# mees/hulc2

Measured on AMD Instinct MI355X. Metric: play-sequences/sec/node (seq_len=32, 200x200 RGB), higher is better.
Workload: dtype bf16; 1 GPU; BASELINE configs[1]: synthetic CALVIN-shaped batch, Hulc2.training_step fwd+bwd+allreduce+Adam, static CNN 200x200 + gripper CNN 84x84, lang = random (B,384) embeddings, dropout 0.1, gripper_control on; sequences_per_gpu_step=64, seq_len=32, parallelism=dp1, launch=hipGraph replay (fwd+bwd graph, all-reduce, optimizer graph), frames=fp32 NCHW, already transformed (the reference's dataloader output), gradient_allreduce=none (one rank, no process group), exact_forward_sites=encfc,goal,head,txl

## Files before the change

### hulc2_amd/csrc/conv_band.h

```cpp
#pragma once
#include "hulc_common.h"

namespace hulc_band {

#define BAND_MAXCLS 4
struct BandCls {
    int OH, OW;
    long y_off;
    int co_base;
    long w_row0;
    long w_tap_off[16];
};
struct BandP {
    const void* X; void* Y; const void* Wt; const float* bias; const void* mask;
    const void* add;
    void* Y16;
    int x_dtype, y_dtype, w_dtype, mask_dtype;
    int Nimg, H, W;
    int OHmax, OWmax;
    int pad_y, pad_x;
    int R;
    int F;
    long x_sn, x_sy, x_sx;
    long y_sn, y_sy, y_sx;
    long ldw;
    int relu;
    unsigned* bits_out;
    const unsigned* bits_in;
    int bshift; long bplane;
    BandCls cls[BAND_MAXCLS];
};

HULC_DEVICE uint4 band_load_bits(const void* X, long off) { return *(const uint4*)((const uint16_t*)X + off); }
template <bool XF32>
HULC_DEVICE uint4 band_load_x(const void* X, long off) {
    if (!XF32) return band_load_bits(X, off);
    const float4* q = (const float4*)((const float*)X + off);
    const float4 a = q[0], c = q[1];
    return make_uint4(pack_bf16x2(a.x, a.y), pack_bf16x2(a.z, a.w), pack_bf16x2(c.x, c.y), pack_bf16x2(c.z, c.w));
}

int launch_band_planes(BandP& p, int NSET, int TH, int TW, hipStream_t s);

}
```

### hulc2_amd/csrc/conv_band.hip

```cpp
#include "hulc_common.h"
#include "hulc_abi_internal.h"
#include "conv_band.h"
#include <stdlib.h>

using namespace hulc_band;

namespace {

template <int C, int NSET, int TH, int TW, int S, int MAXCH, bool MULTI, bool XF32, int BITS, bool STAMP = false>
__global__ __launch_bounds__(512) void conv_band_kernel(BandP p, unsigned long long* stamps = nullptr) {
    constexpr int NT = 512;
    constexpr int K = TH * TW * C, KSTEPS = K / 16;
    constexpr int PS = C * 2 + 16;
    constexpr int WPS = 8 / NSET;
    constexpr int CPP = C / 8;
    static_assert(NT % CPP == 0, "a thread keeps one channel chunk");
    extern __shared__ __attribute__((aligned(16))) char band0[];

    const int tid = threadIdx.x, lane = tid & 63, wave = __builtin_amdgcn_readfirstlane(tid >> 6);
    const int r = lane & 31, h = lane >> 5;
    const int set = wave % NSET, part = wave / NSET;
    const BandCls& cl = p.cls[set];
    const int cl_OH = __builtin_amdgcn_readfirstlane(cl.OH), cl_OW = __builtin_amdgcn_readfirstlane(cl.OW);
    const int cl_co = __builtin_amdgcn_readfirstlane(cl.co_base);
    const long cl_yoff = (long)(((unsigned long long)(unsigned)__builtin_amdgcn_readfirstlane((int)((unsigned long long)cl.y_off >> 32)) << 32) |
                                (unsigned)__builtin_amdgcn_readfirstlane((int)(unsigned)cl.y_off));
    const int Wb = (p.OWmax - 1) * S + TW;
    const float inv_Wb = __builtin_amdgcn_rcpf((float)Wb), inv_OW = __builtin_amdgcn_rcpf((float)cl_OW);
    const int bands = (p.OHmax + p.R - 1) / p.R;
    const int nunits = MULTI ? (p.Nimg + p.F - 1) / p.F : p.Nimg * bands;

    const int cc = tid % CPP;
    uint4 pre[MAXCH];
    unsigned pre_live = 0;
    auto band_rows = [&](int unit, int& n, int& fu, int& r0, int& R, int& rows) {
        if (MULTI) { n = unit * p.F; fu = n + p.F <= p.Nimg ? p.F : p.Nimg - n; r0 = 0; R = p.OHmax; }
        else { n = unit / bands; fu = 1; const int b = unit % bands; r0 = b * p.R; R = (r0 + p.R <= p.OHmax) ? p.R : p.OHmax - r0; }
        rows = (R - 1) * S + TH;
    };
    auto stage_load = [&](int unit) {
        int n, fu, r0, R, rows; band_rows(unit, n, fu, r0, R, rows);
        const int iy0 = r0 * S - p.pad_y, fpx = rows * Wb, npx = fu * fpx;
#pragma unroll
        for (int j = 0; j < MAXCH; ++j) {
            const int px = tid / CPP + j * (NT / CPP);
            int pxc = px < npx ? px : 0, f = 0;
            if (MULTI) { f = fast_div(pxc, __builtin_amdgcn_rcpf((float)fpx)); pxc -= f * fpx; }
            const int br = fast_div(pxc, inv_Wb), bc = pxc - br * Wb;
            const int iy = iy0 + br, ix = bc - p.pad_x;
            const bool inb = px < npx && iy >= 0 && iy < p.H && ix >= 0 && ix < p.W;
            const long off = inb ? (long)(n + f) * p.x_sn + (long)iy * p.x_sy + (long)ix * p.x_sx + cc * 8 : (long)n * p.x_sn;
            pre[j] = band_load_x<XF32>(p.X, off);
            pre_live = j == 0 ? (inb ? 1u : 0u) : (pre_live | ((inb ? 1u : 0u) << j));
        }
    };
    auto stage_store = [&](int unit, char* band) {
        int n, fu, r0, R, rows; band_rows(unit, n, fu, r0, R, rows);
        const int npx = fu * rows * Wb;
        int t2 = tid;
        asm volatile("" : "+v"(t2));
        const int px0 = t2 / CPP, c2 = t2 % CPP;
#pragma unroll
        for (int j = 0; j < MAXCH; ++j) {
            const int px = px0 + j * (NT / CPP);
            if (px < npx) *(uint4*)(band + px * PS + c2 * 16) = ((pre_live >> j) & 1u) ? pre[j] : make_uint4(0, 0, 0, 0);
        }
    };

    constexpr int RPI = 64 / CPP;
    constexpr int WITEMS = (32 / RPI) * TH * TW;
    constexpr int NW = (WITEMS + WPS - 1) / WPS;
    constexpr int WS = K * 2 + 16;
    uint4 wtmp[NW];
    {
        const int wrow = lane / CPP, wc = lane % CPP;
#pragma unroll
        for (int i = 0; i < NW; ++i) {
            const int it = part + i * WPS;
            const int itc = it < WITEMS ? it : WITEMS - 1;
            const int rg = itc / (TH * TW), t = itc % (TH * TW);
            wtmp[i] = band_load_bits(p.Wt, (cl.w_row0 + rg * RPI + wrow) * p.ldw + cl.w_tap_off[t] + wc * 8);
        }
    }
    int unit = blockIdx.x;
    if (unit < nunits) stage_load(unit);
    {
        const int wrow = lane / CPP, wc = lane % CPP;
#pragma unroll
        for (int i = 0; i < NW; ++i) {
            const int it = part + i * WPS;
            if (it < WITEMS) {
                const int rg = it / (TH * TW), t = it % (TH * TW);
                *(uint4*)(band0 + (set * 32 + rg * RPI + wrow) * WS + (t * C + wc * 8) * 2) = wtmp[i];
            }
        }
    }
    __shared__ float sbias[BAND_MAXCLS * 32];
    if (tid < NSET * 32) sbias[tid] = p.bias ? p.bias[p.cls[tid >> 5].co_base + (tid & 31)] : 0.f;
    __syncthreads();
    bf16x8_t wfrag[KSTEPS];
#pragma unroll
    for (int ks = 0; ks < KSTEPS; ++ks) wfrag[ks] = *(const bf16x8_t*)(band0 + (set * 32 + r) * WS + (ks * 16 + h * 8) * 2);
    __builtin_amdgcn_s_waitcnt(0xC07F);
    __syncthreads();

    char* band = band0;
    if (unit < nunits) stage_store(unit, band);
    __syncthreads();
    unsigned long long t_ph[4] = {0, 0, 0, 0}, t_units = 0, c0 = 0, c1 = 0, c2 = 0, c3 = 0;
    for (; unit < nunits; unit += gridDim.x) {
        const int next = unit + gridDim.x;
        const bool have_next = next < nunits;
        if (STAMP) c0 = __builtin_readcyclecounter();
        const bool stagger = MULTI && BITS != 2;
        if (have_next && !stagger) stage_load(next);

        int n, fu, r0, R, rows; band_rows(unit, n, fu, r0, R, rows);
        const int Rc = r0 < cl_OH ? ((r0 + R <= cl_OH) ? R : cl_OH - r0) : 0;
        const int fpix = Rc * cl_OW, npix = fu * fpix;
        const int ntile = (npix + 31) / 32;
        const int my_tiles = ntile > part ? (ntile - part + WPS - 1) / WPS : 0;
        const int slot = (wave * my_tiles) >> 3;
        bool issued = !have_next || !stagger;
        int it = 0;
        if (STAMP) c1 = __builtin_readcyclecounter();
        for (int tile = part; tile < ntile; tile += WPS, ++it) {
            if (!issued && it == slot) { stage_load(next); issued = true; }
            int q = tile * 32 + r;
            const bool live = q < npix;
            if (!live) q = npix - 1;
            int f = 0;
            if (MULTI) { f = fast_div(q, __builtin_amdgcn_rcpf((float)fpix)); q -= f * fpix; }
            const int oy = fast_div(q, inv_OW), ox = q - oy * cl_OW;
            const char* a0 = band + ((f * rows + oy * S) * Wb + ox * S) * PS + h * 16;
            f32x16_t acc;
#pragma unroll
            for (int g = 0; g < 4; ++g) {
                const float4 bv = *(const float4*)(sbias + set * 32 + 8 * g + 4 * h);
                acc[4 * g] = bv.x; acc[4 * g + 1] = bv.y; acc[4 * g + 2] = bv.z; acc[4 * g + 3] = bv.w;
            }
            unsigned mb_in = 0;
            if (BITS == 2) {
                const long pix_off = cl_yoff + (long)(n + f) * p.y_sn + (long)(r0 + oy) * p.y_sy + (long)ox * p.y_sx;
                mb_in = p.bits_in[(long)(cl_co >> 5) * p.bplane + (pix_off >> p.bshift)];
            }
            constexpr int RD = KSTEPS <= 16 ? 8 : 4;
            auto frag = [&](int ks) {
                const int k0 = ks * 16;
                const int t = k0 / C, c0 = k0 % C;
                const int ty = t / TW, tx = t % TW;
                return *(const bf16x8_t*)(a0 + (ty * Wb + tx) * PS + c0 * 2);
            };
            bf16x8_t pf[RD];
#pragma unroll
            for (int i = 0; i < RD; ++i) pf[i] = frag(i);
#pragma unroll
            for (int ks = 0; ks < KSTEPS; ++ks) {
                const bf16x8_t px = pf[ks % RD];
                acc = __builtin_amdgcn_mfma_f32_32x32x16_bf16(wfrag[ks], px, acc, 0, 0, 0);
                __builtin_amdgcn_sched_barrier(0);
                if (ks + RD < KSTEPS) pf[ks % RD] = frag(ks + RD);
                __builtin_amdgcn_sched_barrier(0);
            }
            const long off0 = cl_yoff + (long)(n + f) * p.y_sn + (long)(r0 + oy) * p.y_sy + (long)ox * p.y_sx + cl_co;
            if (p.y_dtype == HULC_BF16) {
                uint2 pk[4];
                unsigned mb_out = 0;
                const uint32_t floor2 = p.relu ? 0u : 0x80008000u;
#pragma unroll
                for (int g = 0; g < 4; ++g) {
                    float v[4] = {acc[4 * g], acc[4 * g + 1], acc[4 * g + 2], acc[4 * g + 3]};
                    if (p.add) {
                        const uint2 a = *(const uint2*)((const uint16_t*)p.add + off0 + 8 * g + 4 * h);
                        v[0] += __uint_as_float(a.x << 16); v[1] += __uint_as_float(a.x & 0xffff0000u);
                        v[2] += __uint_as_float(a.y << 16); v[3] += __uint_as_float(a.y & 0xffff0000u);
                    }
                    pk[g] = make_uint2(max_s16x2(pack_bf16x2(v[0], v[1]), floor2), max_s16x2(pack_bf16x2(v[2], v[3]), floor2));
                }
#pragma unroll
                for (int gp = 0; gp < 2; ++gp) {
                    const auto sx = __builtin_amdgcn_permlane32_swap(pk[2 * gp].x, pk[2 * gp + 1].x, false, false);
                    const auto sy = __builtin_amdgcn_permlane32_swap(pk[2 * gp].y, pk[2 * gp + 1].y, false, false);
                    uint32_t o[4] = {sx[0], sy[0], sx[1], sy[1]};
                    const long off = off0 + 16 * gp + 8 * h;
                    if (BITS == 2) {
#pragma unroll
                        for (int e = 0; e < 4; ++e) o[e] = keep_u16x2(o[e], (mb_in >> (16 * gp + 8 * h + 2 * e)) & 3u);
                    } else if (p.mask) {
                        const uint4 m = *(const uint4*)((const uint16_t*)p.mask + off);
                        const uint32_t mw[4] = {m.x, m.y, m.z, m.w};
#pragma unroll
                        for (int e = 0; e < 4; ++e) {
                            if (!(__uint_as_float(mw[e] << 16) > 0.f)) o[e] &= 0xffff0000u;
                            if (!(__uint_as_float(mw[e] & 0xffff0000u) > 0.f)) o[e] &= 0x0000ffffu;
                        }
                    }
                    if (BITS == 1) {
                        const unsigned a = nonzero_u16x2(o[0]) | (nonzero_u16x2(o[1]) << 2) | (nonzero_u16x2(o[2]) << 4) | (nonzero_u16x2(o[3]) << 6);
                        mb_out |= ((a | (a >> 15)) & 0xffu) << (16 * gp);
                    }
                    if (live) *(uint4*)((uint16_t*)p.Y + off) = make_uint4(o[0], o[1], o[2], o[3]);
                }
                if (BITS == 1) {
                    mb_out <<= 8 * h;
                    const auto other = __builtin_amdgcn_permlane32_swap(mb_out, mb_out, false, false);
                    mb_out |= other[1];
                    if (live && h == 0) p.bits_out[(long)(cl_co >> 5) * p.bplane + ((off0 - cl_co) >> p.bshift)] = mb_out;
                }
            } else {
              if (live) {
                const long off = off0 + 4 * h;
#pragma unroll
                for (int g = 0; g < 4; ++g) {
                    float v[4] = {acc[4 * g], acc[4 * g + 1], acc[4 * g + 2], acc[4 * g + 3]};
                    if (p.relu) {
#pragma unroll
                        for (int e = 0; e < 4; ++e) v[e] = fmaxf(v[e], 0.f);
                    }
                    if (p.mask) {
                        const uint2 m = *(const uint2*)((const uint16_t*)p.mask + off + 8 * g);
                        if (!(__uint_as_float(m.x << 16) > 0.f)) v[0] = 0.f;
                        if (!(__uint_as_float(m.x & 0xffff0000u) > 0.f)) v[1] = 0.f;
                        if (!(__uint_as_float(m.y << 16) > 0.f)) v[2] = 0.f;
                        if (!(__uint_as_float(m.y & 0xffff0000u) > 0.f)) v[3] = 0.f;
                    }
                    *(float4*)((float*)p.Y + off + 8 * g) = make_float4(v[0], v[1], v[2], v[3]);
                    if (p.Y16) *(uint2*)((uint16_t*)p.Y16 + off + 8 * g) = make_uint2(pack_bf16x2(v[0], v[1]), pack_bf16x2(v[2], v[3]));
                }
              }
            }
        }
        if (!issued) stage_load(next);
        if (STAMP) c2 = __builtin_readcyclecounter();
        __syncthreads();
        if (STAMP) c3 = __builtin_readcyclecounter();
        if (have_next) stage_store(next, band);
        __syncthreads();
        if (STAMP) {
            const unsigned long long c4 = __builtin_readcyclecounter();
            t_ph[0] += c1 - c0; t_ph[1] += c2 - c1; t_ph[2] += c3 - c2; t_ph[3] += c4 - c3; t_units += 1;
        }
    }
    if (STAMP && stamps && lane == 0) {
        unsigned long long* o = stamps + ((long)blockIdx.x * 8 + wave) * 5;
#pragma unroll
        for (int e = 0; e < 4; ++e) o[e] = t_ph[e];
        o[4] = t_units;
    }
}

template <int C, int NSET, int TH, int TW, int S, int MAXCH, bool XF32, int BITS>
int launch_band_x(BandP& p, hipStream_t s) {
    constexpr int PS = C * 2 + 16, CPP = C / 8;
    const int Wb = (p.OWmax - 1) * S + TW;
    const long budget = (160 * 1024 - 1024) / 16 * 16;
    const long max_px = (long)MAXCH * (512 / CPP);
    int R = p.OHmax;
    auto px_of = [&](int rr) { return (long)((rr - 1) * S + TH) * Wb; };
    while (R > 1 && (px_of(R) * PS > budget || px_of(R) > max_px)) --R;
    if (px_of(R) * PS > budget || px_of(R) > max_px) return -1;
    int F = 1, nunits;
    if (R == p.OHmax) {
        while (F < p.Nimg && px_of(R) * (F + 1) * PS <= budget && px_of(R) * (F + 1) <= max_px) ++F;
        nunits = (p.Nimg + F - 1) / F;
    } else {
        const int bands = (p.OHmax + R - 1) / R;
        R = (p.OHmax + bands - 1) / bands;
        nunits = p.Nimg * bands;
    }
    p.R = R; p.F = F;
    if ((long)F * R * p.OWmax < 128) return -1;
    size_t lds = ((size_t)px_of(R) * F * PS + 15) / 16 * 16;
    const size_t wbytes = (size_t)NSET * 32 * (TH * TW * C * 2 + 16);
    if (lds < wbytes) lds = wbytes;
    const int per = (nunits + 255) / 256;
    const int grid = (nunits + per - 1) / per;
    if (F > 1) {
        auto kern = conv_band_kernel<C, NSET, TH, TW, S, MAXCH, true, XF32, BITS>;
        static bool attr_set = false;
        if (!attr_set) {
            if (hipFuncSetAttribute((const void*)kern, hipFuncAttributeMaxDynamicSharedMemorySize, 160 * 1024 - 512) != hipSuccess) return -2;
            attr_set = true;
        }
        kern<<<grid, 512, lds, s>>>(p, nullptr);
    } else {
        auto kern = conv_band_kernel<C, NSET, TH, TW, S, MAXCH, false, XF32, BITS>;
        static bool attr_set = false;
        if (!attr_set) {
            if (hipFuncSetAttribute((const void*)kern, hipFuncAttributeMaxDynamicSharedMemorySize, 160 * 1024 - 512) != hipSuccess) return -2;
            attr_set = true;
        }
        const char* se = getenv("HULC_BANDK_STAMPS");
        if (se && *se && C == 32 && !XF32 && BITS == 1) {
            auto kst = conv_band_kernel<C, NSET, TH, TW, S, MAXCH, false, XF32, BITS, true>;
            static bool st_attr = false;
            if (!st_attr) {
                if (hipFuncSetAttribute((const void*)kst, hipFuncAttributeMaxDynamicSharedMemorySize, 160 * 1024 - 512) != hipSuccess) return -2;
                st_attr = true;
            }
            kst<<<grid, 512, lds, s>>>(p, (unsigned long long*)strtoull(se, nullptr, 0));
        } else
        kern<<<grid, 512, lds, s>>>(p, nullptr);
    }
    return 0;
}


constexpr int GLDS_BAND_BYTES = 68 * 1024;
template <int NSET, int TH, int TW, int BITS, bool PAD>
__global__ __launch_bounds__(512) void conv_band_glds_kernel(BandP p) {
    constexpr int C = 64, NT = 512;
    constexpr int K = TH * TW * C, KSTEPS = K / 16, CPP = 8, WPS = 8 / NSET;
    constexpr int SPA = NSET / 2;
    constexpr int BANDB = GLDS_BAND_BYTES;
    __shared__ __attribute__((aligned(2048))) float sbias[BAND_MAXCLS * 32 + 384];
    __shared__ __attribute__((aligned(256))) char bandA_[BANDB];
    __shared__ __attribute__((aligned(256))) char bandB_[BANDB];
    constexpr int MAXTW = BITS == 2 ? (NSET == 2 ? 6 : 12) : 1;
    __shared__ unsigned smask[8][MAXTW][32];
    const int tid = threadIdx.x, lane = tid & 63, wave = __builtin_amdgcn_readfirstlane(tid >> 6);
    const int r = lane & 31, h = lane >> 5;
    const int set = wave % NSET, part = wave / NSET;
    const BandCls& cl = p.cls[set];
    const int cl_OH = cl.OH, cl_OW = cl.OW, cl_co = cl.co_base;
    const long cl_yoff = cl.y_off;
    const int Wb = p.W;
    const float inv_OW = __builtin_amdgcn_rcpf((float)cl_OW);
    const int nunits = p.Nimg;
    const int P = p.H * p.W, NSLOT = P * CPP, NINS = (NSLOT + 63) / 64;
    const int npix = cl_OH * cl_OW, ntile = (npix + 31) / 32;

    constexpr int RPI = 64 / CPP, WITEMS = (32 / RPI) * TH * TW, NW = (WITEMS + WPS - 1) / WPS, WS = K * 2 + 16;
    static_assert((long)SPA * 32 * WS <= BANDB, "the parked weights fit a band array");
    char* const wpark = ((set / SPA) ? bandB_ : bandA_) + (set % SPA) * 32 * WS;
    uint4 wtmp[NW];
    {
        const int wrow = lane / CPP, wc = lane % CPP;
#pragma unroll
        for (int i = 0; i < NW; ++i) {
            const int it = part + i * WPS, itc = it < WITEMS ? it : WITEMS - 1;
            const int rg = itc / (TH * TW), t = itc % (TH * TW);
            wtmp[i] = band_load_bits(p.Wt, (cl.w_row0 + rg * RPI + wrow) * p.ldw + cl.w_tap_off[t] + wc * 8);
        }
#pragma unroll
        for (int i = 0; i < NW; ++i) {
            const int it = part + i * WPS;
            if (it < WITEMS) {
                const int rg = it / (TH * TW), t = it % (TH * TW);
                *(uint4*)(wpark + (rg * RPI + wrow) * WS + (t * C + wc * 8) * 2) = wtmp[i];
            }
        }
    }
    if (tid < NSET * 32) sbias[tid] = p.bias ? p.bias[p.cls[tid >> 5].co_base + (tid & 31)] : 0.f;
    __syncthreads();
    bf16x8_t wfrag[KSTEPS];
#pragma unroll
    for (int ks = 0; ks < KSTEPS; ++ks) wfrag[ks] = *(const bf16x8_t*)(wpark + r * WS + (ks * 16 + h * 8) * 2);
    __builtin_amdgcn_s_waitcnt(0xC07F);
    __syncthreads();
    if (PAD && tid < 16) *(uint4*)((tid < 8 ? bandA_ : bandB_) + P * 128 + (tid & 7) * 16) = make_uint4(0u, 0u, 0u, 0u);

    auto glds_band = [&](int unit, char* band) {
        const uint16_t* frame = (const uint16_t*)p.X + (long)unit * p.x_sn;
        for (int i = wave; i < NINS; i += 8) {
            const int slot = i * 64 + lane;
            if (slot < NSLOT) {
                const int q = slot >> 3, j = slot & 7, c = j ^ ((q >> 1) & 7);
                __builtin_amdgcn_global_load_lds((const void __attribute__((address_space(1)))*)(frame + (long)q * C + c * 8),
                                                 (void __attribute__((address_space(3)))*)(band + i * 1024), 16, 0, 0);
            }
        }
    };
    unsigned mbn[MAXTW];
    auto mask_park = [&]() {
        if (BITS == 2 && lane < 32) {
#pragma unroll
            for (int i = 0; i < MAXTW; ++i) smask[wave][i][lane] = mbn[i];
        }
    };
    auto mask_fetch = [&](int unit) {
#pragma unroll
        for (int i = 0; i < MAXTW; ++i) {
            const int tile = part + i * WPS;
            int q = tile * 32 + r;
            q = q < npix ? q : npix - 1;
            if (tile >= ntile) q = 0;
            const int oy = fast_div(q, inv_OW), ox = q - oy * cl_OW;
            const long pix_off = cl_yoff + (long)unit * p.y_sn + (long)oy * p.y_sy + (long)ox * p.y_sx;
            mbn[i] = p.bits_in[(long)(cl_co >> 5) * p.bplane + (pix_off >> p.bshift)];
        }
    };

    int unit = blockIdx.x;
    if (BITS == 2 && unit < nunits) mask_fetch(unit);
    if (unit < nunits) glds_band(unit, bandA_);
    __builtin_amdgcn_s_waitcnt(0x0F70);
    mask_park();
    __builtin_amdgcn_s_waitcnt(0xC07F);
    __builtin_amdgcn_s_barrier();
    auto do_unit = [&](int unit, const char* __restrict__ band, char* __restrict__ band_next) {
        const int next = unit + gridDim.x;
        if (BITS == 2 && next < nunits) mask_fetch(next);
        if (next < nunits) glds_band(next, band_next);

        auto do_tile = [&](int tile, unsigned mb_in) {
            int q = tile * 32 + r;
            const bool live = q < npix;
            if (!live) q = npix - 1;
            const int oy = fast_div(q, inv_OW), ox = q - oy * cl_OW;
            int rowq[TH], colq[TW];
#pragma unroll
            for (int ty = 0; ty < TH; ++ty) { const int iy = oy + ty - p.pad_y; rowq[ty] = (!PAD || (iy >= 0 && iy < p.H)) ? iy * Wb : -0x40000000; }
#pragma unroll
            for (int tx = 0; tx < TW; ++tx) { const int ix = ox + tx - p.pad_x; colq[tx] = (!PAD || (ix >= 0 && ix < p.W)) ? ix : -0x40000000; }
            f32x16_t acc;
#pragma unroll
            for (int g = 0; g < 4; ++g) {
                const float4 bv = *(const float4*)(sbias + set * 32 + 8 * g + 4 * h);
                acc[4 * g] = bv.x; acc[4 * g + 1] = bv.y; acc[4 * g + 2] = bv.z; acc[4 * g + 3] = bv.w;
            }
            constexpr int RD = 8;
            auto frag = [&](int ks) {
                const int k0 = ks * 16, t = k0 / C, kc = (k0 % C) / 16;
                const int ty = t / TW, tx = t % TW;
                int qs = rowq[ty] + colq[tx];
                if (PAD) qs = qs < 0 ? P : qs;
                const unsigned u = (unsigned)qs << 3;
                const unsigned off = (u << 4) + ((((unsigned)(2 * kc) + (unsigned)h) << 4) ^ (u & 0x70u));
                return *(const bf16x8_t*)(band + off);
            };
            bf16x8_t pf[RD];
#pragma unroll
            for (int i = 0; i < RD; ++i) pf[i] = frag(i);
#pragma unroll
            for (int ks = 0; ks < KSTEPS; ++ks) {
                const bf16x8_t px = pf[ks % RD];
                acc = __builtin_amdgcn_mfma_f32_32x32x16_bf16(wfrag[ks], px, acc, 0, 0, 0);
                __builtin_amdgcn_sched_barrier(0);
                if (ks + RD < KSTEPS) pf[ks % RD] = frag(ks + RD);
                __builtin_amdgcn_sched_barrier(0);
            }
            const long off0 = cl_yoff + (long)unit * p.y_sn + (long)oy * p.y_sy + (long)ox * p.y_sx + cl_co;
            uint2 pk[4];
            const uint32_t floor2 = p.relu ? 0u : 0x80008000u;
#pragma unroll
            for (int g = 0; g < 4; ++g)
                pk[g] = make_uint2(max_s16x2(pack_bf16x2(acc[4 * g], acc[4 * g + 1]), floor2), max_s16x2(pack_bf16x2(acc[4 * g + 2], acc[4 * g + 3]), floor2));
#pragma unroll
            for (int gp = 0; gp < 2; ++gp) {
                const auto sx = __builtin_amdgcn_permlane32_swap(pk[2 * gp].x, pk[2 * gp + 1].x, false, false);
                const auto sy = __builtin_amdgcn_permlane32_swap(pk[2 * gp].y, pk[2 * gp + 1].y, false, false);
                uint32_t o[4] = {sx[0], sy[0], sx[1], sy[1]};
                if (BITS == 2) {
#pragma unroll
                    for (int e = 0; e < 4; ++e) o[e] = keep_u16x2(o[e], (mb_in >> (16 * gp + 8 * h + 2 * e)) & 3u);
                }
                if (live) *(uint4*)((uint16_t*)p.Y + off0 + 16 * gp + 8 * h) = make_uint4(o[0], o[1], o[2], o[3]);
            }
        };
        int ti = 0;
        for (int tile = part; tile < ntile; tile += WPS, ++ti) do_tile(tile, BITS == 2 ? smask[wave][ti][r] : 0u);
        __builtin_amdgcn_s_waitcnt(0x0F70);
        if (next < nunits) mask_park();
        __builtin_amdgcn_s_barrier();
    };
    for (; unit < nunits; unit += 2 * gridDim.x) {
        do_unit(unit, bandA_, bandB_);
        if (unit + (int)gridDim.x < nunits) do_unit(unit + gridDim.x, bandB_, bandA_);
    }
}

template <int NSET, int TH, int TW, int BITS, bool PAD>
int launch_band_glds(BandP& p, hipStream_t s) {
    const long P = (long)p.H * p.W + (PAD ? 1 : 0);
    if ((P * 128 + 1023) / 1024 * 1024 > GLDS_BAND_BYTES) return -1;
    const long npix = (long)p.OHmax * p.OWmax;
    if (BITS == 2 && (npix + 31) / 32 > (long)(NSET == 2 ? 6 : 12) * (8 / NSET)) return -1;
    const size_t lds = 0;
    const int nunits = p.Nimg, per = (nunits + 255) / 256, grid = (nunits + per - 1) / per;
    auto kern = conv_band_glds_kernel<NSET, TH, TW, BITS, PAD>;
    kern<<<grid, 512, lds, s>>>(p);
    return 0;
}

template <int C, int NSET, int TH, int TW, int S, int MAXCH, int BITS_OK>
int launch_band(BandP& p, hipStream_t s) {
    const int want = p.bits_out ? 1 : (p.bits_in ? 2 : 0);
    if (want && want != BITS_OK) return -1;
    if (want) {
        constexpr int B = BITS_OK ? BITS_OK : 1;
        return p.x_dtype == HULC_F32 ? launch_band_x<C, NSET, TH, TW, S, MAXCH, true, B>(p, s) : launch_band_x<C, NSET, TH, TW, S, MAXCH, false, B>(p, s);
    }
    return p.x_dtype == HULC_F32 ? launch_band_x<C, NSET, TH, TW, S, MAXCH, true, 0>(p, s) : launch_band_x<C, NSET, TH, TW, S, MAXCH, false, 0>(p, s);
}

inline bool mask_only(const void* mask, const unsigned* bits_in) { return mask != nullptr && bits_in == nullptr; }

}

int hulc_conv_band_dispatch(int C, int NSET, int TH, int TW, int S, const void* x, int x_dtype, int N, int H, int W, int pad_y, int pad_x,
                            long x_sn, long x_sy, long x_sx, void* y, int y_dtype, long y_sn, long y_sy, long y_sx, const void* wt,
                            int w_dtype, long ldw, const float* bias, const void* mask, int mask_dtype, int relu, int ncls,
                            const int* cls_OH, const int* cls_OW, const long* cls_yoff, const int* cls_cobase, const long* cls_wrow0,
                            const long* cls_wtap , const void* add, unsigned* bits_out, const unsigned* bits_in, int bits_channels,
                            void* y16, hipStream_t s) {
    if (ncls != NSET || ncls > BAND_MAXCLS || TH * TW > 16) return 1;
    if (y16 && ((y_dtype != HULC_F32 && y_dtype != HULC_F16) || mask || add || bits_out || bits_in)) return 1;
    if (y_dtype == HULC_F16 && !y16) return 1;
    BandP p;
    p.X = x; p.Y = y; p.Wt = wt; p.bias = bias; p.mask = mask; p.add = add; p.Y16 = y16;
    p.bits_out = bits_out; p.bits_in = bits_in; p.bshift = 0; p.bplane = 0;
    if (bits_out || bits_in) {
        if (y_dtype != HULC_BF16 || (bits_channels != 32 && bits_channels != 64 && bits_channels != 128) || y_sx % bits_channels || y_sy % bits_channels ||
            y_sn % bits_channels) return 1;
        for (int c = 0; c < ncls; ++c) if (cls_yoff[c] % bits_channels) return 1;
        while ((1 << p.bshift) < bits_channels) ++p.bshift;
        p.bplane = (long)N * y_sn / bits_channels;
    }
    if (add && y_dtype != HULC_BF16) return 1;
    if (bits_out && !relu) return 1;
    if (w_dtype != HULC_BF16 || (mask && mask_dtype != HULC_BF16)) return 1;
    p.x_dtype = x_dtype; p.y_dtype = y_dtype; p.w_dtype = w_dtype; p.mask_dtype = mask_dtype;
    p.Nimg = N; p.H = H; p.W = W; p.pad_y = pad_y; p.pad_x = pad_x; p.R = 1; p.F = 1;
    p.x_sn = x_sn; p.x_sy = x_sy; p.x_sx = x_sx; p.y_sn = y_sn; p.y_sy = y_sy; p.y_sx = y_sx;
    p.ldw = ldw; p.relu = relu;
    p.OHmax = 0; p.OWmax = 0;
    for (int c = 0; c < ncls; ++c) {
        p.cls[c].OH = cls_OH[c]; p.cls[c].OW = cls_OW[c]; p.cls[c].y_off = cls_yoff[c]; p.cls[c].co_base = cls_cobase[c];
        p.cls[c].w_row0 = cls_wrow0[c];
        for (int t = 0; t < 16; ++t) p.cls[c].w_tap_off[t] = t < TH * TW ? cls_wtap[c * 16 + t] : 0;
        if (cls_OH[c] > p.OHmax) p.OHmax = cls_OH[c];
        if (cls_OW[c] > p.OWmax) p.OWmax = cls_OW[c];
    }
    int rc = 1;
    if (y_dtype == HULC_F16 && !(C == 64 && S == 1 && NSET == 2 && TH == 3 && TW == 3)) return 1;
    if (C == 32 && NSET == 2 && TH == 4 && TW == 4 && S == 2) rc = launch_band<32, 2, 4, 4, 2, 12, 1>(p, s);
    else if (C == 64 && S == 1 && ((NSET == 2 && TH == 3 && TW == 3) || (NSET == 4 && TH == 2 && TW == 2))) {
        rc = -1;
        if (NSET == 2 && TH == 3 && TW == 3) rc = launch_band_planes(p, NSET, TH, TW, s);
        if (rc == -1 && y_dtype == HULC_F16) return 1;
        const bool contiguous = x_sx == 64 && x_sy == (long)W * 64 && x_sn == (long)H * W * 64 && ((uintptr_t)x % 16) == 0;
        if (rc == -1 && !mask_only(mask, bits_in) && !add && !bits_out && x_dtype == HULC_BF16 && y_dtype == HULC_BF16 && contiguous &&
            (long)p.OHmax * p.OWmax >= 256) {
            const bool padded = pad_y != 0 || pad_x != 0;
            if (NSET == 2 && !padded && !bits_in) rc = launch_band_glds<2, 3, 3, 0, false>(p, s);
            else if (NSET == 2 && padded && bits_in) rc = launch_band_glds<2, 3, 3, 2, true>(p, s);
            else if (NSET == 4 && padded && bits_in) rc = launch_band_glds<4, 2, 2, 2, true>(p, s);
        }
        if (rc == -1) rc = NSET == 2 ? launch_band<64, 2, 3, 3, 1, 10, 2>(p, s) : launch_band<64, 4, 2, 2, 1, 12, 2>(p, s);
    }
    else return 1;
    if (rc == -1) return 1;
    if (rc < 0) return hulc_fail(-8, "conv band: could not raise the dynamic LDS limit");
    return 0;
}
```

Baseline: 21270 play-sequences/s.

## Add shape-specialized conv2 data-gradient kernel with double-buffered LDS bands and register-resident weights

Adds a dedicated kernel for the 23x23 to 49x49 stride-2 transposed conv (conv2 dgrad, 4 sub-pixel classes). Weights are parked in LDS once and kept in registers. Input frames are double-buffered in LDS via global_load_lds so the next image's load overlaps the current image's MFMA tiles. Masks are prefetched per unit and outputs are staged through swizzled LDS for coalesced stores. It is used only when the exact shape, stride and dtype checks pass, and otherwise falls back to the generic band kernel. It adds a large hard-coded path plus an optional cycle-stamp profiling mode.

```diff
diff --git a/hulc2_amd/csrc/conv2_dgrad.hip b/hulc2_amd/csrc/conv2_dgrad.hip
--- /dev/null
+++ b/hulc2_amd/csrc/conv2_dgrad.hip
@@ -0,0 +1,247 @@
+#include "hulc_common.h"
+#include "hulc_abi_internal.h"
+#include "conv_band.h"
+#include <stdlib.h>
+
+using namespace hulc_band;
+
+namespace {
+
+constexpr int D2_HIN = 23, D2_WIN = 23;
+constexpr int D2_HO = 49, D2_WO = 49, D2_CO = 32;
+constexpr int D2_P = D2_HIN * D2_WIN;
+constexpr int D2_NBLK = (D2_P + 1 + 7) / 8;
+constexpr int D2_BAND_BYTES = D2_NBLK * 1024;
+constexpr int D2_PW = (D2_WO + 1) / 2;
+constexpr int D2_MAXT = 5;
+constexpr int D2_STG = 16 * 128;
+
+template <bool STAMP = false>
+__global__ __launch_bounds__(512) void conv2_dgrad_kernel(BandP p, unsigned long long* stamps = nullptr) {
+    constexpr int C = 64, TAPS = 4, K = TAPS * C, KSTEPS = K / 16, CPP = 8;
+    __shared__ __attribute__((aligned(4096))) unsigned smask[8][2 * D2_MAXT][32];
+    __shared__ __attribute__((aligned(256))) char bandA_[D2_BAND_BYTES];
+    __shared__ __attribute__((aligned(256))) char bandB_[D2_BAND_BYTES];
+    __shared__ __attribute__((aligned(256))) char stage_[8][D2_STG];
+    const int tid = threadIdx.x, lane = tid & 63, wave = __builtin_amdgcn_readfirstlane(tid >> 6);
+    const int r = lane & 31, h = lane >> 5;
+    const int py = wave & 1, part = wave >> 1;
+    const int nrow = D2_HO / 2 + 1 - py, npair = nrow * D2_PW, ntile = (npair + 31) / 32;
+    const float inv_PW = __builtin_amdgcn_rcpf((float)D2_PW);
+    const int nunits = p.Nimg;
+    char* const stg = stage_[wave];
+
+    constexpr int RPI = 64 / CPP, WITEMS = 4 * (32 / RPI) * TAPS, NW = WITEMS / 8, WS = K * 2 + 16;
+    static_assert(4 * 32 * WS <= D2_BAND_BYTES, "the parked weights fit a band array");
+    {
+        uint4 wtmp[NW];
+        const int wrow = lane / CPP, wc = lane % CPP;
+#pragma unroll
+        for (int i = 0; i < NW; ++i) {
+            const int it = wave + i * 8, c = it / ((32 / RPI) * TAPS), rg = (it / TAPS) % (32 / RPI), t = it % TAPS;
+            wtmp[i] = band_load_bits(p.Wt, (p.cls[c].w_row0 + rg * RPI + wrow) * p.ldw + p.cls[c].w_tap_off[t] + wc * 8);
+        }
+#pragma unroll
+        for (int i = 0; i < NW; ++i) {
+            const int it = wave + i * 8, c = it / ((32 / RPI) * TAPS), rg = (it / TAPS) % (32 / RPI), t = it % TAPS;
+            *(uint4*)(bandA_ + (c * 32 + rg * RPI + wrow) * WS + (t * C + wc * 8) * 2) = wtmp[i];
+        }
+    }
+    __syncthreads();
+    bf16x8_t wf0[KSTEPS], wf1[KSTEPS];
+#pragma unroll
+    for (int ks = 0; ks < KSTEPS; ++ks) {
+        wf0[ks] = *(const bf16x8_t*)(bandA_ + ((2 * py) * 32 + r) * WS + (ks * 16 + h * 8) * 2);
+        wf1[ks] = *(const bf16x8_t*)(bandA_ + ((2 * py + 1) * 32 + r) * WS + (ks * 16 + h * 8) * 2);
+    }
+    __builtin_amdgcn_s_waitcnt(0xC07F);
+    __syncthreads();
+    if (tid < 16) {
+        char* b = tid < 8 ? bandA_ : bandB_;
+        *(uint4*)(b + (D2_P >> 3) * 1024 + ((tid & 7) << 7) + (D2_P & 7) * 16) = make_uint4(0u, 0u, 0u, 0u);
+    }
+
+    auto glds_one = [&](int unit, char* band, int i) {
+        const uint16_t* frame = (const uint16_t*)p.X + (long)unit * p.x_sn;
+        const int slot = lane >> 3, pj = lane & 7, q = i * 8 + pj;
+        if (i < D2_NBLK && q < D2_P)
+            __builtin_amdgcn_global_load_lds((const void __attribute__((address_space(1)))*)(frame + (long)q * C + ((slot ^ (i & 1)) << 3)),
+                                             (void __attribute__((address_space(3)))*)(band + i * 1024), 16, 0, 0);
+    };
+    unsigned mbn[2 * D2_MAXT];
+    int moff[2 * D2_MAXT];
+#pragma unroll
+    for (int i = 0; i < D2_MAXT; ++i) {
+        const int tile = part + i * 4;
+        int q = tile * 32 + r;
+        q = q < npair ? q : npair - 1;
+        if (tile >= ntile) q = 0;
+        const int iy = fast_div(q, inv_PW), jx = q - iy * D2_PW;
+        const int pix = (2 * iy + py) * D2_WO + 2 * jx;
+        moff[2 * i] = pix;
+        moff[2 * i + 1] = 2 * jx + 1 < D2_WO ? pix + 1 : pix;
+    }
+    const long unit_words = p.y_sn >> p.bshift;
+    auto mask_fetch = [&](int unit) {
+        const unsigned* mp = p.bits_in + (long)unit * unit_words;
+#pragma unroll
+        for (int i = 0; i < 2 * D2_MAXT; ++i) mbn[i] = mp[moff[i]];
+    };
+    auto mask_park = [&]() {
+        if (lane < 32) {
+#pragma unroll
+            for (int i = 0; i < 2 * D2_MAXT; ++i) smask[wave][i][lane] = mbn[i];
+        }
+    };
+
+    int unit = blockIdx.x;
+    if (unit < nunits) {
+        mask_fetch(unit);
+        for (int i = wave; i < D2_NBLK; i += 8) glds_one(unit, bandA_, i);
+    }
+    __builtin_amdgcn_s_waitcnt(0x0F70);
+    mask_park();
+    __builtin_amdgcn_s_waitcnt(0xC07F);
+    __builtin_amdgcn_s_barrier();
+    unsigned long long t_issue = 0, t_tiles = 0, t_wait = 0, t_bar = 0, t_units = 0;
+    auto do_unit = [&](int unit, const char* __restrict__ band, char* __restrict__ band_next) {
+        const int next = unit + gridDim.x;
+        unsigned long long c0 = 0, c1 = 0, c2 = 0, c3 = 0;
+        if (STAMP) c0 = __builtin_readcyclecounter();
+        if (next < nunits) mask_fetch(next);
+        if (STAMP) c1 = __builtin_readcyclecounter();
+        uint16_t* const yu = (uint16_t*)p.Y + (long)unit * p.y_sn;
+
+        auto do_tile = [&](int tile, unsigned mb0, unsigned mb1) {
+            int q = tile * 32 + r;
+            if (q >= npair) q = npair - 1;
+            const int iy = fast_div(q, inv_PW), jx = q - iy * D2_PW;
+            const char* tap_base[TAPS];
+#pragma unroll
+            for (int ty = 0; ty < 2; ++ty)
+#pragma unroll
+                for (int tx = 0; tx < 2; ++tx) {
+                    const int sy = iy + ty - 1, sx = jx + tx - 1;
+                    const int qt = (sy >= 0 && sy < D2_HIN && sx >= 0 && sx < D2_WIN) ? sy * D2_WIN + sx : D2_P;
+                    const int blk = qt >> 3;
+                    tap_base[ty * 2 + tx] = band + blk * 1024 + ((h ^ (blk & 1)) << 7) + ((qt & 7) << 4);
+                }
+            f32x16_t acc0, acc1;
+#pragma unroll
+            for (int e = 0; e < 16; ++e) { acc0[e] = 0.f; acc1[e] = 0.f; }
+            constexpr int RD = 4;
+            auto frag = [&](int ks) { return *(const bf16x8_t*)(tap_base[ks / 4] + (ks % 4) * 256); };
+            bf16x8_t pf[RD];
+#pragma unroll
+            for (int i = 0; i < RD; ++i) pf[i] = frag(i);
+#pragma unroll
+            for (int ks = 0; ks < KSTEPS; ++ks) {
+                const bf16x8_t px = pf[ks % RD];
+                acc0 = __builtin_amdgcn_mfma_f32_32x32x16_bf16(wf0[ks], px, acc0, 0, 0, 0);
+                acc1 = __builtin_amdgcn_mfma_f32_32x32x16_bf16(wf1[ks], px, acc1, 0, 0, 0);
+                __builtin_amdgcn_sched_barrier(0);
+                if (ks + RD < KSTEPS) pf[ks % RD] = frag(ks + RD);
+                __builtin_amdgcn_sched_barrier(0);
+            }
+            const uint32_t floor2 = p.relu ? 0u : 0x80008000u;
+            uint4 o[2][2];
+#pragma unroll
+            for (int c = 0; c < 2; ++c) {
+                const f32x16_t& a = c ? acc1 : acc0;
+                const unsigned mb = c ? mb1 : mb0;
+                uint2 pk[4];
+#pragma unroll
+                for (int g = 0; g < 4; ++g)
+                    pk[g] = make_uint2(max_s16x2(pack_bf16x2(a[4 * g], a[4 * g + 1]), floor2), max_s16x2(pack_bf16x2(a[4 * g + 2], a[4 * g + 3]), floor2));
+#pragma unroll
+                for (int gp = 0; gp < 2; ++gp) {
+                    const auto sx = __builtin_amdgcn_permlane32_swap(pk[2 * gp].x, pk[2 * gp + 1].x, false, false);
+                    const auto sy = __builtin_amdgcn_permlane32_swap(pk[2 * gp].y, pk[2 * gp + 1].y, false, false);
+                    uint32_t w[4] = {sx[0], sy[0], sx[1], sy[1]};
+#pragma unroll
+                    for (int e = 0; e < 4; ++e) w[e] = keep_u16x2(w[e], (mb >> (16 * gp + 8 * h + 2 * e)) & 3u);
+                    o[c][gp] = make_uint4(w[0], w[1], w[2], w[3]);
+                }
+            }
+#pragma unroll
+            for (int m = 0; m < 2; ++m) {
+                if ((r >> 4) == m) {
+                    const int l = r & 15;
+#pragma unroll
+                    for (int c = 0; c < 2; ++c)
+#pragma unroll
+                        for (int gp = 0; gp < 2; ++gp)
+                            *(uint4*)(stg + l * 128 + (((4 * c + 2 * gp + h) ^ (l & 7)) << 4)) = o[c][gp];
+                }
+                asm volatile("" ::: "memory");
+                const int j = lane & 7, l0 = lane >> 3, l1 = 8 + (lane >> 3);
+                const uint4 v0 = *(const uint4*)(stg + l0 * 128 + ((j ^ (l0 & 7)) << 4));
+                const uint4 v1 = *(const uint4*)(stg + l1 * 128 + ((j ^ (l1 & 7)) << 4));
+#pragma unroll
+                for (int k = 0; k < 2; ++k) {
+                    const int l = k ? l1 : l0;
+                    const int qs = tile * 32 + 16 * m + l;
+                    const int sy = fast_div(qs, inv_PW), sx = qs - sy * D2_PW;
+                    if (qs < npair && (j < 4 || 2 * sx + 1 < D2_WO))
+                        *(uint4*)(yu + ((2 * sy + py) * D2_WO + 2 * sx) * D2_CO + j * 8) = k ? v1 : v0;
+                }
+            }
+        };
+        int ti = 0, li = wave;
+        constexpr int PER_TILE = 2;
+        for (int tile = part; tile < ntile; tile += 4, ++ti) {
+            if (next < nunits) {
+#pragma unroll
+                for (int k = 0; k < PER_TILE; ++k, li += 8) glds_one(next, band_next, li);
+            }
+            do_tile(tile, smask[wave][2 * ti][r], smask[wave][2 * ti + 1][r]);
+        }
+        if (next < nunits)
+            for (; li < D2_NBLK; li += 8) glds_one(next, band_next, li);
+        if (STAMP) c2 = __builtin_readcyclecounter();
+        __builtin_amdgcn_s_waitcnt(0x0F70);
+        if (STAMP) c3 = __builtin_readcyclecounter();
+        if (next < nunits) mask_park();
+        __builtin_amdgcn_s_barrier();
+        if (STAMP) {
+            const unsigned long long c4 = __builtin_readcyclecounter();
+            t_issue += c1 - c0; t_tiles += c2 - c1; t_wait += c3 - c2; t_bar += c4 - c3; t_units += 1;
+        }
+    };
+    for (; unit < nunits; unit += 2 * gridDim.x) {
+        do_unit(unit, bandA_, bandB_);
+        if (unit + (int)gridDim.x < nunits) do_unit(unit + gridDim.x, bandB_, bandA_);
+    }
+    if (STAMP && stamps && lane == 0) {
+        unsigned long long* o = stamps + ((long)blockIdx.x * 8 + wave) * 5;
+        o[0] = t_issue; o[1] = t_tiles; o[2] = t_wait; o[3] = t_bar; o[4] = t_units;
+    }
+}
+
+}
+
+namespace hulc_band {
+
+int launch_conv2_dgrad(BandP& p, hipStream_t s) {
+    if (p.x_dtype != HULC_BF16 || p.y_dtype != HULC_BF16 || p.w_dtype != HULC_BF16 || !p.bits_in || p.bits_out || p.add || p.Y16 || p.bias)
+        return -1;
+    if (p.H != D2_HIN || p.W != D2_WIN || p.pad_y != 1 || p.pad_x != 1) return -1;
+    if (p.x_sx != 64 || p.x_sy != (long)D2_WIN * 64 || p.x_sn != (long)D2_P * 64 || ((uintptr_t)p.X % 16) != 0) return -1;
+    if (p.y_sx != 2 * D2_CO || p.y_sy != 2L * D2_WO * D2_CO || p.y_sn != (long)D2_HO * D2_WO * D2_CO || ((uintptr_t)p.Y % 16) != 0) return -1;
+    if (p.bshift != 5) return -1;
+    for (int c = 0; c < 4; ++c) {
+        const int cy = c >> 1, cx = c & 1;
+        if (p.cls[c].OH != (D2_HO + 1) / 2 - cy || p.cls[c].OW != (D2_WO + 1) / 2 - cx || p.cls[c].y_off != (long)(cy * D2_WO + cx) * D2_CO ||
+            p.cls[c].co_base != 0) return -1;
+    }
+    const int nunits = p.Nimg, per = (nunits + 255) / 256, grid = (nunits + per - 1) / per;
+    const char* se = getenv("HULC_D2_STAMPS");
+    if (se && *se) {
+        conv2_dgrad_kernel<true><<<grid, 512, 0, s>>>(p, (unsigned long long*)strtoull(se, nullptr, 0));
+        return 0;
+    }
+    conv2_dgrad_kernel<><<<grid, 512, 0, s>>>(p);
+    return 0;
+}
+
+}
diff --git a/hulc2_amd/csrc/conv_band.h b/hulc2_amd/csrc/conv_band.h
--- a/hulc2_amd/csrc/conv_band.h
+++ b/hulc2_amd/csrc/conv_band.h
@@ -41,5 +41,6 @@
 }
 
 int launch_band_planes(BandP& p, int NSET, int TH, int TW, hipStream_t s);
+int launch_conv2_dgrad(BandP& p, hipStream_t s);
 
 }
diff --git a/hulc2_amd/csrc/conv_band.hip b/hulc2_amd/csrc/conv_band.hip
--- a/hulc2_amd/csrc/conv_band.hip
+++ b/hulc2_amd/csrc/conv_band.hip
@@ -545,7 +545,10 @@
             const bool padded = pad_y != 0 || pad_x != 0;
             if (NSET == 2 && !padded && !bits_in) rc = launch_band_glds<2, 3, 3, 0, false>(p, s);
             else if (NSET == 2 && padded && bits_in) rc = launch_band_glds<2, 3, 3, 2, true>(p, s);
-            else if (NSET == 4 && padded && bits_in) rc = launch_band_glds<4, 2, 2, 2, true>(p, s);
+            else if (NSET == 4 && padded && bits_in) {
+                rc = launch_conv2_dgrad(p, s);
+                if (rc == -1) rc = launch_band_glds<4, 2, 2, 2, true>(p, s);
+            }
         }
         if (rc == -1) rc = NSET == 2 ? launch_band<64, 2, 3, 3, 1, 10, 2>(p, s) : launch_band<64, 4, 2, 2, 1, 12, 2>(p, s);
     }
```

Result: no change. 21330 play-sequences/s (median of 6 runs) (+0.3%).
